# fishaudio/fish-diffusion

Measured on NVIDIA H100. Metric: mel_frames_per_sec_100step_ddpm, higher is better.
Workload: dtype f32 (3x fp16 split-product wgmma, fp32 accumulate)

## Files before the change

### fish_diffusion_b200/csrc/fd_common.cuh

```cuda
#pragma once
#include <cuda_runtime.h>
#include <cuda_fp16.h>
#include <cuda_bf16.h>
#include <stdint.h>

#define FD_F16 0
#define FD_BF16 1
#define FD_SINGLE 0x10

#define FD_MAX_SEG 16

#define FD_EPI_LINEAR 0
#define FD_EPI_GATE 1
#define FD_EPI_RES_SKIP 2
#define FD_EPI_MAG 3
#define FD_EPI_GATE_BWD 4

#define FD_ACT_NONE 0
#define FD_ACT_RELU 1
#define FD_ACT_LRELU 2
#define FD_ACT_GELU 3

struct FdSeg {
  int src;
// ... 123 lines not shown
  const float sg = fd_sigmoid(g), th = fd_tanh(f);
  dg = dz * th * sg * (1.f - sg);
  df = dz * sg * (1.f - th * th);
}

__device__ __forceinline__ void fd_split2(float a, float b, int prec, uint32_t& hi2, uint32_t& lo2) {
  if (prec == FD_F16) {
    asm("cvt.rn.satfinite.f16x2.f32 %0, %1, %2;" : "=r"(hi2) : "f"(b), "f"(a));
    const float2 hf = __half22float2(*reinterpret_cast<const __half2*>(&hi2));
    asm("cvt.rn.satfinite.f16x2.f32 %0, %1, %2;" : "=r"(lo2) : "f"(b - hf.y), "f"(a - hf.x));
  } else {
    asm("cvt.rn.satfinite.bf16x2.f32 %0, %1, %2;" : "=r"(hi2) : "f"(b), "f"(a));
    const float ha = __uint_as_float(hi2 << 16), hb = __uint_as_float(hi2 & 0xffff0000u);
    asm("cvt.rn.satfinite.bf16x2.f32 %0, %1, %2;" : "=r"(lo2) : "f"(b - hb), "f"(a - ha));
  }
}

template <int V>
__device__ __forceinline__ void fd_store_planes(uint16_t* planes, size_t plane_elems, size_t off,
                                                const float (&y)[V], int prec) {
  uint32_t hi[V / 2], lo[V / 2];
#pragma unroll
  for (int i = 0; i < V / 2; ++i) fd_split2(y[2 * i], y[2 * i + 1], prec, hi[i], lo[i]);
  if (V == 4) {
    *reinterpret_cast<uint2*>(planes + off) = make_uint2(hi[0], hi[1]);
    *reinterpret_cast<uint2*>(planes + plane_elems + off) = make_uint2(lo[0], lo[1]);
  } else {
    *reinterpret_cast<uint4*>(planes + off) = make_uint4(hi[0], hi[1], hi[2 % (V / 2)], hi[3 % (V / 2)]);
    *reinterpret_cast<uint4*>(planes + plane_elems + off) = make_uint4(lo[0], lo[1], lo[2 % (V / 2)], lo[3 % (V / 2)]);
  }
}

template <int V>
__device__ __forceinline__ void fd_load_planes(const uint16_t* planes, size_t plane_elems, size_t off,
                                               float (&y)[V], int prec) {
  uint32_t hi[4], lo[4];
  if (V == 4) {
    const uint2 a = *reinterpret_cast<const uint2*>(planes + off);
    const uint2 b = *reinterpret_cast<const uint2*>(planes + plane_elems + off);
    hi[0] = a.x; hi[1] = a.y; lo[0] = b.x; lo[1] = b.y;
  } else {
    const uint4 a = *reinterpret_cast<const uint4*>(planes + off);
    const uint4 b = *reinterpret_cast<const uint4*>(planes + plane_elems + off);
    hi[0] = a.x; hi[1] = a.y; hi[2] = a.z; hi[3] = a.w; lo[0] = b.x; lo[1] = b.y; lo[2] = b.z; lo[3] = b.w;
  }
#pragma unroll
  for (int i = 0; i < V / 2; ++i) fd_combine2(hi[i], lo[i], prec, y[2 * i], y[2 * i + 1]);
}

__device__ __forceinline__ void fd_load_hi8(const uint16_t* planes, size_t off, float (&y)[8], int prec) {
  const uint4 a = *reinterpret_cast<const uint4*>(planes + off);
  const uint32_t w[4] = {a.x, a.y, a.z, a.w};
#pragma unroll
  for (int i = 0; i < 4; ++i) {
    y[2 * i] = fd_h2f((uint16_t)(w[i] & 0xffff), prec);
    y[2 * i + 1] = fd_h2f((uint16_t)(w[i] >> 16), prec);
  }
}

template <int V>
__device__ __forceinline__ void fd_load_f32(const float* p, float (&y)[V]) {
#pragma unroll
  for (int i = 0; i < V; i += 4) {
    float4 q = *reinterpret_cast<const float4*>(p + i);
    y[i] = q.x; y[i + 1] = q.y; y[i + 2] = q.z; y[i + 3] = q.w;
  }
}
template <int V>
__device__ __forceinline__ void fd_store_f32(float* p, const float (&y)[V]) {
#pragma unroll
  for (int i = 0; i < V; i += 4)
    *reinterpret_cast<float4*>(p + i) = make_float4(y[i], y[i + 1], y[i + 2], y[i + 3]);
}

template <typename I>
struct FdRows {
  I item;
  int t0, dt, nrows;
  __device__ __forceinline__ I row(const FdTapGemm& p, int r) const { return item + (I)min(t0 + r * dt, p.T - 1); }
};
// ... 55 lines not shown
    for (int i = 0; i < V; ++i) a[r][i] = (a[r][i] * p.acc_scale + bias[i] + pre[r][i]) * p.post_scale;
  if (p.out_f32 != nullptr && p.out_accum) {
#pragma unroll
    for (int r = 0; r < R; ++r) {
      float v[V];
      fd_load_f32<V>(p.out_f32 + off[r], v);
#pragma unroll
      for (int i = 0; i < V; ++i) a[r][i] += v[i];
    }
  }
  const float slope = p.act == FD_ACT_NONE ? 1.f : p.act == FD_ACT_RELU ? 0.f : p.act_slope;
#pragma unroll
  for (int r = 0; r < R; ++r) {
    if (r >= rw.nrows) break;
    if ((masked >> r) & 1u) {
#pragma unroll
      for (int i = 0; i < V; ++i) a[r][i] = 0.f;
    }
    if (p.out_f32 != nullptr) fd_store_f32<V>(p.out_f32 + off[r], a[r]);
    if (p.out_planes != nullptr) {
      float v[V];
      if (p.act == FD_ACT_GELU) {
#pragma unroll
        for (int i = 0; i < V; ++i) v[i] = fd_gelu(a[r][i] * p.planes_scale);
      } else {
#pragma unroll
        for (int i = 0; i < V; ++i) v[i] = fd_act(a[r][i] * p.planes_scale, slope);
      }
      fd_store_planes<V>(p.out_planes, plane, off[r], v, prec);
    }
  }
}

template <int R, int V, int PREC, typename I>
__device__ __forceinline__ void fd_epi_res_skip(const FdTapGemm& p, const FdRows<I>& rw, int n, bool is_res,
                                                const float (&a)[R][V], const float (&bias)[V]) {
  const int prec = PREC < 0 ? p.prec : PREC;
  const size_t plane = (size_t)p.B * p.T * p.C;
  const I cn = (I)(is_res ? n : n - p.C);
  I off[R];
#pragma unroll
  for (int r = 0; r < R; ++r) off[r] = rw.row(p, r) * (I)p.C + cn;
  if (is_res) {
    if (p.last_layer) return;
    float x[R][V];
#pragma unroll
    for (int r = 0; r < R; ++r) fd_load_planes<V>(p.x_planes, plane, off[r], x[r], prec);
    uint16_t* const xo = p.x_out_planes != nullptr ? p.x_out_planes : p.x_planes;
#pragma unroll
    for (int r = 0; r < R; ++r) {
      if (r >= rw.nrows) break;
#pragma unroll
      for (int i = 0; i < V; ++i) x[r][i] = (x[r][i] + (a[r][i] * p.acc_scale + bias[i])) * 0.70710678118654752440f;
      fd_store_planes<V>(xo, plane, off[r], x[r], prec);
    }
  } else {
    float sk[R][V];
    if (!p.first_layer) {
#pragma unroll
      for (int r = 0; r < R; ++r) fd_load_f32<V>(p.skip_f32 + off[r], sk[r]);
    }
#pragma unroll
    for (int r = 0; r < R; ++r) {
      if (r >= rw.nrows) break;
      float y[V];
#pragma unroll
      for (int i = 0; i < V; ++i) {
        y[i] = a[r][i] * p.acc_scale + bias[i];
        if (!p.first_layer) y[i] += sk[r][i];
      }
      if (p.last_layer) {
#pragma unroll
        for (int i = 0; i < V; ++i) y[i] *= p.skip_scale;
        fd_store_planes<V>(p.skip_planes, plane, off[r], y, prec);
      } else {
        fd_store_f32<V>(p.skip_f32 + off[r], y);
      }
    }
  }
}

template <int V>
__device__ __forceinline__ void fd_epi_gate(const FdTapGemm& p, int t, float (&g)[V], float (&f)[V], float (&z)[V],
                                            const float (&bias)[2][V], const float (&add)[2][V],
                                            const float (&lo)[2][V], const float (&hi)[2][V]) {
#pragma unroll
  for (int i = 0; i < V; ++i) {
    g[i] = g[i] * p.acc_scale + bias[0][i];
    f[i] = f[i] * p.acc_scale + bias[1][i];
  }
  if (p.addend != nullptr) {
#pragma unroll
    for (int i = 0; i < V; ++i) { g[i] += add[0][i]; f[i] += add[1][i]; }
  }
  if (t < p.dil) {
#pragma unroll
    for (int i = 0; i < V; ++i) { g[i] -= lo[0][i]; f[i] -= lo[1][i]; }
  }
  if (t + p.dil >= p.T) {
#pragma unroll
    for (int i = 0; i < V; ++i) { g[i] -= hi[0][i]; f[i] -= hi[1][i]; }
  }
#pragma unroll
  for (int i = 0; i < V; ++i) z[i] = fd_sigmoid(g[i]) * fd_tanh(f[i]);
}

template <int V>
struct FdColSums {
  float all[2][V], lo[2][V], hi[2][V];
};

template <int R, int V, int PREC, typename I>
// ... 120 lines not shown
```

### fish_diffusion_b200/csrc/fd_tapgemm_simt.cu

```cuda
#include "fd_common.cuh"

namespace {

constexpr int BM = 128;
constexpr int BK = 16;
constexpr int APITCH = BM + 4;

template <int RUN, int EPI>
__global__ void __launch_bounds__(256) fd_tapgemm_simt_kernel(const FdTapGemm p) {
  constexpr int BN = 2 * RUN;
  constexpr int TXC = RUN / 4;
  constexpr int TYC = 256 / TXC;
  constexpr int RM = BM / TYC;
  constexpr int BPITCH = BN + 4;

  __shared__ float As[BK][APITCH];
  __shared__ float Bs[BK][BPITCH];

  const int tid = threadIdx.x;
  const int tx = tid % TXC, ty = tid / TXC;
  const int tiles_t = (p.T + BM - 1) / BM;
  const int m_tile = blockIdx.x;
  const int b = m_tile / tiles_t;
  const int t0 = (m_tile % tiles_t) * BM;
  const int j = blockIdx.y;

  int run0, run1;
  if (EPI == FD_EPI_GATE || EPI == FD_EPI_MAG) {
    run0 = fd_gate_col(p, j * RUN);
    run1 = run0 + p.gate_tile / 2;
  } else {
    run0 = j * BN;
    run1 = run0 + RUN;
  }

  float acc[RM][8];
#pragma unroll
  for (int r = 0; r < RM; ++r)
#pragma unroll
    for (int c = 0; c < 8; ++c) acc[r][c] = 0.f;

  const size_t w_plane = (size_t)p.n_total * p.k_total;
  int koff = 0;
  for (int s = 0; s < p.num_seg; ++s) {
    const FdSeg sg = p.seg[s];
    const uint16_t* src = p.src[sg.src];
    const size_t a_plane = (size_t)p.src_ps[sg.src];
    const size_t a_rs = (size_t)p.src_rs[sg.src], a_bs = (size_t)p.src_bs[sg.src];
    for (int k0 = 0; k0 < sg.k_len; k0 += BK) {
      {
        const int row = tid % BM, kh = tid / BM;
        const int t = t0 + row + sg.shift;
        float v[8];
        const int kk = k0 + kh * 8;
        if (t >= 0 && t < p.T && t0 + row < p.T && kk < sg.k_len) {
          const size_t off = (size_t)b * a_bs + (size_t)t * a_rs + sg.c_off + kk;
          if (p.single) fd_load_hi8(src, off, v, p.prec);
          else fd_load_planes<8>(src, a_plane, off, v, p.prec);
        } else {
#pragma unroll
          for (int i = 0; i < 8; ++i) v[i] = 0.f;
        }
#pragma unroll
        for (int i = 0; i < 8; ++i) As[kh * 8 + i][row] = v[i];
      }
// ... 79 lines not shown
          float a[1][4] = {{acc[r][4 * h], acc[r][4 * h + 1], acc[r][4 * h + 2], acc[r][4 * h + 3]}};
          fd_epi_gate_bwd<1, 4, -1>(p, FdRows<size_t>{(size_t)b * p.T, tr + r, 1, 1}, n, a, s);
        }
        fd_gate_bwd_colsums<TXC>(p, s, t0 < p.dil, t0 + BM + p.dil > p.T, tid % 32 < TXC && n < p.n_total, b, n);
      } else {
        if (n >= p.n_total) continue;
#pragma unroll
        for (int r = 0; r < RM; ++r) {
          if (r >= nrows) break;
          float bias[4];
#pragma unroll
          for (int i = 0; i < 4; ++i) bias[i] = p.bias != nullptr ? p.bias[(size_t)b * p.bias_bstride + n + i] : 0.f;
          float a[1][4] = {{acc[r][4 * h], acc[r][4 * h + 1], acc[r][4 * h + 2], acc[r][4 * h + 3]}};
          const FdRows<size_t> row{(size_t)b * p.T, tr + r, 1, 1};
          if constexpr (EPI == FD_EPI_LINEAR) fd_epi_linear<1, 4, -1>(p, row, n, a, bias);
          else fd_epi_res_skip<1, 4, -1>(p, row, n, n < p.C, a, bias);
        }
      }
    }
  }
}

template <int RUN>
int launch_run(const FdTapGemm& p, cudaStream_t stream) {
  const int tiles_t = (p.T + BM - 1) / BM;
  dim3 grid(p.B * tiles_t, 1, 1), block(256);
  if (p.epi == FD_EPI_GATE) {
    grid.y = (p.n_total / 2 + RUN - 1) / RUN;
    fd_tapgemm_simt_kernel<RUN, FD_EPI_GATE><<<grid, block, 0, stream>>>(p);
  } else if (p.epi == FD_EPI_MAG) {
    grid.y = (p.n_total / 2 + RUN - 1) / RUN;
    fd_tapgemm_simt_kernel<RUN, FD_EPI_MAG><<<grid, block, 0, stream>>>(p);
  } else if (p.epi == FD_EPI_RES_SKIP) {
    grid.y = (p.n_total + 2 * RUN - 1) / (2 * RUN);
    fd_tapgemm_simt_kernel<RUN, FD_EPI_RES_SKIP><<<grid, block, 0, stream>>>(p);
  } else if (p.epi == FD_EPI_GATE_BWD) {
    grid.y = (p.n_total + 2 * RUN - 1) / (2 * RUN);
    fd_tapgemm_simt_kernel<RUN, FD_EPI_GATE_BWD><<<grid, block, 0, stream>>>(p);
  } else {
    grid.y = (p.n_total + 2 * RUN - 1) / (2 * RUN);
    fd_tapgemm_simt_kernel<RUN, FD_EPI_LINEAR><<<grid, block, 0, stream>>>(p);
  }
  FD_CHECK_CUDA(cudaGetLastError());
  return 0;
}

constexpr int WG_R = 64, WG_C = 64, WG_T = 16;

__global__ void __launch_bounds__(256) fd_wgrad_simt_kernel(const FdWgradK p, const uint16_t* row0,
                                                            const uint16_t* row1, const uint16_t* col0,
                                                            const uint16_t* col1, int prec, int single) {
  static_assert(WG_R == WG_C, "rows and columns share the staging code");
  __shared__ __align__(16) float Rs[WG_T][WG_R + 4];
  __shared__ __align__(16) float Cs[WG_T][WG_C + 4];
  const int tid = threadIdx.x;
  const int s = blockIdx.z, r0 = blockIdx.y * WG_R, c0 = blockIdx.x * WG_C;

  const bool is_col = tid >= 128;
  const int grp = tid % 8, tl = (tid % 128) / 8;
  const int i = (is_col ? c0 : r0) + grp * 8;
  const uint16_t* src = nullptr;
  int C = 0, ch = 0, shift = 0;
  if (!is_col) {
    for (int g = 0; g < p.num_row_seg; ++g)
      if (i >= p.row_start[g] && i < p.row_start[g] + p.row_width[g]) {
        src = p.row_src[g] == 0 ? row0 : row1;
        C = p.row_C[p.row_src[g]]; ch = p.row_coff[g] + (i - p.row_start[g]);
// ... 94 lines not shown
```

### fish_diffusion_b200/csrc/fd_tapgemm_tc.cu

```cuda
#include <cuda.h>
#include "fd_common.cuh"
#include "fd_host.h"
#include "fd_tc_ptx.cuh"

namespace {

constexpr int BLOCK_M = 128;

template <int BLOCK_N, int BLOCK_K, int EPI, int NPL>
struct Cfg {
  static constexpr bool PP = EPI == FD_EPI_GATE || EPI == FD_EPI_RES_SKIP;
  static constexpr int ROWS = PP ? 64 : BLOCK_M;
  static constexpr int A_BYTES = ROWS * BLOCK_K * 2;
  static constexpr int W_BYTES = BLOCK_N * BLOCK_K * 2;
  static constexpr int GROUP = BLOCK_K >= 64 || PP ? 1 : 64 / BLOCK_K;
  static constexpr int SUB_BYTES = NPL * (A_BYTES + W_BYTES);
  static constexpr int STAGE_BYTES = GROUP * SUB_BYTES;
  static constexpr int TX_BYTES = SUB_BYTES;
  static constexpr int SWIZZLE_BYTES = BLOCK_K * 2;
  static constexpr uint32_t SWIZZLE_MODE = swizzle_mode_for(SWIZZLE_BYTES);
  static constexpr uint32_t SBO = 8 * SWIZZLE_BYTES;
  static constexpr int BIAS_FLOATS = (EPI == FD_EPI_GATE ? 3 : 1) * BLOCK_N;
  static constexpr int BIAS_TOTAL = (PP ? 2 : 1) * BIAS_FLOATS;
  static constexpr int NUM_STAGES = fd_tc_frame_stages(STAGE_BYTES, BIAS_TOTAL);
  static constexpr int SMEM_BYTES = fd_tc_frame_bytes(NUM_STAGES, STAGE_BYTES, BIAS_TOTAL);
  static_assert(NUM_STAGES >= 2, "pipeline needs at least two stages");
  static_assert(SMEM_BYTES <= FD_TC_SMEM_BUDGET, "shared memory");
};

template <int BLOCK_N, int EPI>
__device__ __forceinline__ void stage_bias(const FdTapGemm& p, int b, int n0, float* bias_s, int i0, int step) {
  if (EPI == FD_EPI_GATE) {
    const size_t bo = (size_t)b * p.gbias_bstride + n0;
    for (int i = i0; i < BLOCK_N; i += step) {
      bias_s[i] = p.gbias_full[bo + i];
      bias_s[BLOCK_N + i] = p.gbias_lo[bo + i];
      bias_s[2 * BLOCK_N + i] = p.gbias_hi[bo + i];
    }
  } else {
    for (int i = i0; i < BLOCK_N; i += step)
      bias_s[i] = p.bias ? p.bias[(size_t)b * p.bias_bstride + n0 + i] : 0.f;
  }
}
template <int EPI>
__device__ __forceinline__ long long bias_key(const FdTapGemm& p, int b, int n0) {
  return EPI == FD_EPI_GATE ? (long long)b * p.gbias_bstride + n0 : (long long)b * p.bias_bstride + n0;
}

template <int BLOCK_N, int EPI, int PREC>
__device__ __forceinline__ void tile_epilogue(const FdTapGemm& p, const float* acc, int b, int n_tile, int rw0,
                                              const float* bias_s, uint32_t my_scratch, int lane) {
  const int n0 = n_tile * BLOCK_N;
  if constexpr (EPI == FD_EPI_GATE || EPI == FD_EPI_MAG) {
    constexpr int HALF = BLOCK_N / 2;
    const uint32_t sb = smem_u32(bias_s);
    const int r = lane >> 1, sub = lane & 1;
    const int t = rw0 + r;
    const bool valid = t < p.T;
    const bool e_lo = t < p.dil, e_hi = t + p.dil >= p.T;
    const bool edge_any = __any_sync(0xffffffffu, valid && (e_lo || e_hi));
    const size_t zplane = (size_t)p.B * p.T * p.C, zrow = ((size_t)b * p.T + t) * p.C + (size_t)n_tile * HALF;
    const size_t yplane = (size_t)p.B * p.T * p.n_total, yrow = ((size_t)b * p.T + t) * p.n_total;
#pragma unroll
    for (int c = 0; c < HALF; c += 16) {
      frag_to_scratch<16>(my_scratch, acc, c, 0, lane);
      frag_to_scratch<16>(my_scratch, acc, HALF + c, 16, lane);
      __syncwarp();
      float g[8], f[8];
      {
        const float4 g0 = scratch_ld4(my_scratch, r, 2 * sub), g1 = scratch_ld4(my_scratch, r, 2 * sub + 1);
        const float4 f0 = scratch_ld4(my_scratch, r, 4 + 2 * sub), f1 = scratch_ld4(my_scratch, r, 5 + 2 * sub);
        g[0] = g0.x; g[1] = g0.y; g[2] = g0.z; g[3] = g0.w; g[4] = g1.x; g[5] = g1.y; g[6] = g1.z; g[7] = g1.w;
        f[0] = f0.x; f[1] = f0.y; f[2] = f0.z; f[3] = f0.w; f[4] = f1.x; f[5] = f1.y; f[6] = f1.z; f[7] = f1.w;
      }
      __syncwarp();
      const int cc = c + 8 * sub;
      if (valid) {
        if (EPI == FD_EPI_MAG) {
          fd_epi_mag<8, PREC>(p, b, t, n_tile * HALF + cc, g, f);
        } else {
          float add[2][8], bias[2][8], lo[2][8], hi[2][8], z[8];
          if (p.addend != nullptr) {
#pragma unroll
            for (int h = 0; h < 2; ++h) ldcs_f32(p.addend + yrow + n0 + h * HALF + cc, add[h]);
          }
#pragma unroll
          for (int h = 0; h < 2; ++h) lds_f32(sb + 4u * (h * HALF + cc), bias[h]);
          if (edge_any) {
#pragma unroll
            for (int h = 0; h < 2; ++h)
              if (e_lo) lds_f32(sb + 4u * (BLOCK_N + h * HALF + cc), lo[h]);
#pragma unroll
            for (int h = 0; h < 2; ++h)
              if (e_hi) lds_f32(sb + 4u * (2 * BLOCK_N + h * HALF + cc), hi[h]);
          }
          fd_epi_gate<8>(p, t, g, f, z, bias, add, lo, hi);
          if (p.y_planes != nullptr) {
            const int ng = p.gate_tile == BLOCK_N ? n0 + cc : fd_gate_col(p, n_tile * HALF + cc);
            fd_store_planes<8>(p.y_planes, yplane, yrow + ng, g, PREC);
            fd_store_planes<8>(p.y_planes, yplane, yrow + ng + p.gate_tile / 2, f, PREC);
          }
          fd_store_planes<8>(p.out_planes, zplane, zrow + cc, z, PREC);
        }
      }
    }
  } else if constexpr (BLOCK_N >= 64) {
    const uint32_t bias_addr = smem_u32(bias_s);
    const int j4 = (lane & 7) * 4, rsub = lane >> 3;
    const int rbase = rw0 + rsub;
    const FdRows<uint32_t> rows{(uint32_t)b * (uint32_t)p.T, rbase, 4,
                                rbase < p.T ? min(4, (p.T - rbase + 3) / 4) : 0};
#pragma unroll
    for (int c = 0; c < BLOCK_N; c += 32) {
      const int col = c + j4;
      const int n = n0 + col;
      frag_to_scratch<32>(my_scratch, acc, c, 0, lane);
      __syncwarp();
      float a[4][4];
#pragma unroll
      for (int r = 0; r < 4; ++r) {
        const float4 x = scratch_ld4(my_scratch, 4 * r + rsub, lane & 7);
        a[r][0] = x.x; a[r][1] = x.y; a[r][2] = x.z; a[r][3] = x.w;
      }
      __syncwarp();
      if constexpr (EPI == FD_EPI_GATE_BWD) {
        FdColSums<4> s{};
        fd_epi_gate_bwd<4, 4, PREC>(p, rows, n, a, s);
        fd_gate_bwd_colsums<8>(p, s, rw0 < p.dil, rw0 + 16 + p.dil > p.T, rsub == 0, b, n);
      } else {
        float bias[4];
        lds_f32(bias_addr + 4u * col, bias);
        if constexpr (EPI == FD_EPI_RES_SKIP) fd_epi_res_skip<4, 4, PREC>(p, rows, n, n0 < p.C, a, bias);
        else fd_epi_linear<4, 4, PREC>(p, rows, n, a, bias);
      }
    }
  } else {
    static_assert(EPI == FD_EPI_LINEAR, "narrow tiles: LINEAR only");
    constexpr int PER = BLOCK_N / 2;
    frag_to_scratch<BLOCK_N>(my_scratch, acc, 0, 0, lane);
    __syncwarp();
    const int r = lane >> 1, sub = lane & 1;
    float v[PER];
#pragma unroll
    for (int q4 = 0; q4 < PER / 4; ++q4) {
      const float4 x = scratch_ld4(my_scratch, r, sub * (PER / 4) + q4);
      v[4 * q4] = x.x; v[4 * q4 + 1] = x.y; v[4 * q4 + 2] = x.z; v[4 * q4 + 3] = x.w;
    }
    __syncwarp();
    const int t = rw0 + r;
    const FdRows<uint32_t> row{(uint32_t)b * (uint32_t)p.T, t, 1, t < p.T ? 1 : 0};
#pragma unroll
    for (int h = 0; h < PER / 8; ++h) {
      const int cc = sub * PER + h * 8;
      float a[1][8], bias[8];
#pragma unroll
      for (int i = 0; i < 8; ++i) a[0][i] = v[h * 8 + i];
      lds_f32(smem_u32(bias_s) + 4u * cc, bias);
      fd_epi_linear<1, 8, PREC>(p, row, n0 + cc, a, bias);
    }
  }
}

template <int BLOCK_N, int BLOCK_K, int EPI, int PREC, int NPL>
__global__ void __launch_bounds__(FD_TC_THREADS, 1)
fd_tapgemm_tc_kernel(const __grid_constant__ CUtensorMap tm_src0, const __grid_constant__ CUtensorMap tm_src1,
                     const __grid_constant__ CUtensorMap tm_w, const FdTapGemm p) {
// ... 48 lines not shown

  consumer_regs();
  const int wg = warp / 4;
  const int wq = warp % 4;
  const uint32_t my_scratch = smem_u32(f.scratch) + warp * FD_TC_SCRATCH_WARP_BYTES;
  float* bias_s = f.bias;
  float acc[BLOCK_N / 2];
  long long staged_key = -1;
  for (int tile = blockIdx.x; tile < num_tiles; tile += gridDim.x) {
    const int m_tile = tile / num_n_tiles;
    const int n_tile = (tile % num_n_tiles + m_tile) % num_n_tiles;
    const int b = m_tile / tiles_t, t0 = (m_tile % tiles_t) * BLOCK_M;
    const int n0 = n_tile * BLOCK_N;

    if (EPI == FD_EPI_LINEAR && bias_key<EPI>(p, b, n0) != staged_key) {
      staged_key = bias_key<EPI>(p, b, n0);
      named_bar_sync<1, FD_TC_CONSUMER_THREADS>();
      stage_bias<BLOCK_N, EPI>(p, b, n0, bias_s, threadIdx.x, FD_TC_CONSUMER_THREADS);
      named_bar_sync<1, FD_TC_CONSUMER_THREADS>();
    }

    ring_mainloop(acc, ring, total_k_blocks, C::GROUP, lane, [&](int stage, int nb) {
      for (int g = 0; g < nb; ++g) {
        const uint32_t st = smem_u32(f.ring + stage * C::STAGE_BYTES + g * C::SUB_BYTES);
        const uint32_t wg_a = wg * 64 * C::SWIZZLE_BYTES;
        const uint64_t a_hi = make_smem_desc(st + wg_a, 16, C::SBO, C::SWIZZLE_MODE);
        const uint64_t a_lo = make_smem_desc(st + C::A_BYTES + wg_a, 16, C::SBO, C::SWIZZLE_MODE);
        const uint64_t w_hi = make_smem_desc(st + NPL * C::A_BYTES, 16, C::SBO, C::SWIZZLE_MODE);
        const uint64_t w_lo = make_smem_desc(st + NPL * C::A_BYTES + C::W_BYTES, 16, C::SBO, C::SWIZZLE_MODE);
        split_mma<MMA, NPL, BLOCK_K / 16, 32>(acc, a_hi, a_lo, w_hi, w_lo);
      }
    });

    tile_epilogue<BLOCK_N, EPI, PREC>(p, acc, b, n_tile, t0 + wg * 64 + wq * 16, bias_s, my_scratch, lane);
  }
}

template <int BLOCK_N, int BLOCK_K, int EPI, int PREC, int NPL>
__global__ void __launch_bounds__(FD_TC_THREADS, 1)
fd_tapgemm_pp_kernel(const __grid_constant__ CUtensorMap tm_src0, const __grid_constant__ CUtensorMap tm_src1,
                     const __grid_constant__ CUtensorMap tm_w, const FdTapGemm p) {
  using C = Cfg<BLOCK_N, BLOCK_K, EPI, NPL>;
  static_assert(C::PP && C::GROUP == 1, "ping-pong schedule: GATE / RES_SKIP, one k-block per stage");
  using MMA = Wgmma<BLOCK_N, PREC>;
  extern __shared__ uint8_t smem_raw[];
  const TcFrame f = tc_frame(smem_raw, C::NUM_STAGES, C::STAGE_BYTES, C::BIAS_TOTAL);

  const int warp = threadIdx.x / 32;
  const int lane = threadIdx.x % 32;
  const int rank = (int)cluster_ctarank();
  const int pair = blockIdx.x / 2, num_pairs = gridDim.x / 2;

  const int tiles_t = (p.T + 63) / 64;
  const int num_m_tiles = p.B * tiles_t;
  const int num_n_tiles = p.n_total / BLOCK_N;
  const int num_units = (num_m_tiles + 1) / 2 * num_n_tiles;
  int total_k_blocks = 0;
  for (int sI = 0; sI < p.num_seg; ++sI) total_k_blocks += p.seg[sI].k_len / BLOCK_K;

  tc_prologue<true>(f, C::NUM_STAGES, 2 * 4, &tm_src0, &tm_src1, &tm_w);

  if (warp >= FD_TC_PRODUCER_WARP) {
    producer_regs();
    if (warp == FD_TC_PRODUCER_WARP && lane == 0) {
      Ring ring{f.full, f.empty, C::NUM_STAGES};
      for (int u = pair; u < num_units; u += num_pairs) {
        const int m_pair = u / num_n_tiles;
        const int n_tile = (u % num_n_tiles + m_pair) % num_n_tiles;
        const int m_tile = min(2 * m_pair + rank, num_m_tiles - 1);
        const int b = m_tile / tiles_t, t0 = (m_tile % tiles_t) * 64;
        const int n0 = n_tile * BLOCK_N;
        SegCursor sc;
#pragma unroll 1
        for (int kb = 0; kb < total_k_blocks; ++kb) {
          ring.wait_empty();
          uint8_t* st = f.ring + ring.stage * C::STAGE_BYTES;
          mbar_expect_tx(ring.full_bar(), C::TX_BYTES);
          const FdSeg sg = p.seg[sc.s];
          tma_load_4d(st, sg.src == 0 ? &tm_src0 : &tm_src1, ring.full_bar(), sg.c_off + sc.k0, t0 + sg.shift, b, 0);
          tma_load_3d_multicast(st + NPL * C::A_BYTES + rank * (NPL * C::W_BYTES / 2), &tm_w, ring.full_bar(),
                                sc.koff + sc.k0 + p.w_kshift, n0 + (NPL == 1 ? rank * (BLOCK_N / 2) : 0),
                                NPL == 2 ? rank : 0, 0x3);
          sc.next(BLOCK_K, sg.k_len);
          ring.next();
        }
      }
    }
  } else {
    consumer_regs();
    const int wg = warp / 4;
    const int wq = warp % 4;
    const uint32_t my_scratch = smem_u32(f.scratch) + warp * FD_TC_SCRATCH_WARP_BYTES;
    float* my_bias = f.bias + wg * C::BIAS_FLOATS;
    float acc[BLOCK_N / 2];
    PingPong turn(f.full, f.empty, C::NUM_STAGES, total_k_blocks, wg);
    long long staged_key = -1;
    for (int u = pair + wg * num_pairs; u < num_units; u += 2 * num_pairs) {
      const int m_pair = u / num_n_tiles;
      const int n_tile = (u % num_n_tiles + m_pair) % num_n_tiles;
      const int m_tile = 2 * m_pair + rank;
      const bool valid = m_tile < num_m_tiles;
      const int b = m_tile / tiles_t, t0 = (m_tile % tiles_t) * 64;
      const int n0 = n_tile * BLOCK_N;

      if (valid && bias_key<EPI>(p, b, n0) != staged_key) {
        staged_key = bias_key<EPI>(p, b, n0);
        wg == 0 ? named_bar_sync<3, 128>() : named_bar_sync<4, 128>();
        stage_bias<BLOCK_N, EPI>(p, b, n0, my_bias, threadIdx.x % 128, 128);
        wg == 0 ? named_bar_sync<3, 128>() : named_bar_sync<4, 128>();
      }

      turn.mainloop(acc, u == pair, u + num_pairs < num_units, lane, [&](int stage) {
        const uint32_t st = smem_u32(f.ring + stage * C::STAGE_BYTES);
        const uint64_t a_hi = make_smem_desc(st, 16, C::SBO, C::SWIZZLE_MODE);
        const uint64_t a_lo = make_smem_desc(st + C::A_BYTES, 16, C::SBO, C::SWIZZLE_MODE);
        const uint64_t w_hi = make_smem_desc(st + NPL * C::A_BYTES, 16, C::SBO, C::SWIZZLE_MODE);
        const uint64_t w_lo = make_smem_desc(st + NPL * C::A_BYTES + C::W_BYTES, 16, C::SBO, C::SWIZZLE_MODE);
        split_mma<MMA, NPL, BLOCK_K / 16, 32>(acc, a_hi, a_lo, w_hi, w_lo);
      });

      if (valid) tile_epilogue<BLOCK_N, EPI, PREC>(p, acc, b, n_tile, t0 + wq * 16, my_bias, my_scratch, lane);
    }
  }
  __syncwarp();
  cluster_sync();
}

template <int BLOCK_T>
struct GateTCfg {
  static constexpr int BLOCK_K = 32;
  static constexpr int ROW_BYTES = BLOCK_K * 2;
  static constexpr int ACT_ROWS = BLOCK_T + 16;
  static constexpr int MAX_DIL = (ACT_ROWS - BLOCK_T) / 2;
  static constexpr int ACT_PLANE = ACT_ROWS * ROW_BYTES;
  static constexpr int W_PLANE = 64 * ROW_BYTES;
  static constexpr int W_OFF = 2 * ACT_PLANE;
  static constexpr int STAGE_BYTES = W_OFF + 3 * 2 * W_PLANE;
  static constexpr uint32_t SWIZZLE_MODE = swizzle_mode_for(ROW_BYTES);
  static constexpr uint32_t SBO = 8 * ROW_BYTES;
  static constexpr int NUM_STAGES = fd_tc_frame_stages(STAGE_BYTES, 0);
  static constexpr int SMEM_BYTES = fd_tc_frame_bytes(NUM_STAGES, STAGE_BYTES, 0);
  static_assert(ACT_ROWS <= 256, "one TMA box per plane");
  static_assert(ACT_PLANE % 512 == 0 && STAGE_BYTES % 1024 == 0, "planes start on 64 B swizzle atoms");
  static_assert(NUM_STAGES >= 3, "ring depth");
  static_assert(SMEM_BYTES <= FD_TC_SMEM_BUDGET, "shared memory");
};

template <int BLOCK_T, int PREC>
__device__ __forceinline__ void gate_t_epilogue(const FdTapGemm& p, const float* acc, int b, int t0, int ch,
                                                uint32_t my_scratch, int lane) {
  const int half = p.gate_tile / 2;
  const int e = lane >> 2, q4 = lane & 3;
  const int n_g = fd_gate_col(p, ch) + e, n_f = n_g + half;
  const size_t bo = (size_t)b * p.gbias_bstride;
// ... 153 lines not shown

template <int BLOCK_T, int PREC>
int launch_gate_t(const FdTapGemm& p, cudaStream_t stream) {
  using C = GateTCfg<BLOCK_T>;
  CUtensorMap tmx, tmw;
  int rc = planes_map(&tmx, p.src[0], p.src_C[0], p.T, p.B, p.src_rs[0], p.src_bs[0], p.src_ps[0], C::BLOCK_K,
                      BLOCK_T + 2 * p.dil, 1, "gate_t x");
  if (rc) return rc;
  const int half = p.gate_tile / 2;
  const cuuint64_t K = (cuuint64_t)p.k_total;
  const cuuint64_t dims[5] = {K, 8, 2, (cuuint64_t)p.n_total / 8, 2};
  const cuuint64_t strides[4] = {K * 2, (cuuint64_t)half * K * 2, 8 * K * 2, (cuuint64_t)p.n_total * K * 2};
  const cuuint32_t box[5] = {(cuuint32_t)C::BLOCK_K, 8, 2, 4, 2};
  rc = encode_tiled(&tmw, p.w, 5, dims, strides, box, "gate_t w");
  if (rc) return rc;
  const int units = p.B * ((p.T + BLOCK_T - 1) / BLOCK_T) * (p.n_total / 128);
  return fd_tc_launch<fd_gate_t_kernel<BLOCK_T, PREC>>(C::SMEM_BYTES, 2 * units, stream, false, 2, tmx, tmw, p);
}

template <int BLOCK_N, int BLOCK_K, int EPI, int PREC, int NPL>
int launch_inst(const FdTapGemm& p, cudaStream_t stream) {
  using C = Cfg<BLOCK_N, BLOCK_K, EPI, NPL>;
  CUtensorMap tm0, tm1, tmw;
  int rc = planes_map(&tm0, p.src[0], p.src_C[0], p.T, p.B, p.src_rs[0], p.src_bs[0], p.src_ps[0], BLOCK_K, C::ROWS,
                      NPL, "tapgemm src0");
  if (rc) return rc;
  if (p.src[1] != nullptr) {
    rc = planes_map(&tm1, p.src[1], p.src_C[1], p.T, p.B, p.src_rs[1], p.src_bs[1], p.src_ps[1], BLOCK_K, C::ROWS, NPL,
                    "tapgemm src1");
    if (rc) return rc;
  } else {
    tm1 = tm0;
  }
  const int m_tiles = p.B * ((p.T + C::ROWS - 1) / C::ROWS), n_tiles = p.n_total / BLOCK_N;
  if constexpr (C::PP) {
    rc = weights_map(&tmw, p.w, p.n_total, p.k_total, BLOCK_K, NPL == 2 ? BLOCK_N : BLOCK_N / 2, 1, "tapgemm w");
    if (rc) return rc;
    return fd_tc_launch<fd_tapgemm_pp_kernel<BLOCK_N, BLOCK_K, EPI, PREC, NPL>>(
        C::SMEM_BYTES, 2 * ((m_tiles + 1) / 2 * n_tiles), stream, false, 2, tm0, tm1, tmw, p);
  } else {
    rc = weights_map(&tmw, p.w, p.n_total, p.k_total, BLOCK_K, BLOCK_N, NPL, "tapgemm w");
    if (rc) return rc;
    return fd_tc_launch<fd_tapgemm_tc_kernel<BLOCK_N, BLOCK_K, EPI, PREC, NPL>>(C::SMEM_BYTES, m_tiles * n_tiles,
                                                                              stream, false, 1, tm0, tm1, tmw, p);
  }
}

template <int BLOCK_N, int BLOCK_K, int EPI>
int launch_cfg(const FdTapGemm& p, cudaStream_t stream) {
  if (p.single) {
    return p.prec == FD_F16 ? launch_inst<BLOCK_N, BLOCK_K, EPI, FD_F16, 1>(p, stream)
                            : launch_inst<BLOCK_N, BLOCK_K, EPI, FD_BF16, 1>(p, stream);
  }
  return p.prec == FD_F16 ? launch_inst<BLOCK_N, BLOCK_K, EPI, FD_F16, 2>(p, stream)
                          : launch_inst<BLOCK_N, BLOCK_K, EPI, FD_BF16, 2>(p, stream);
}

template <int BLOCK_N, int BLOCK_K>
int launch_epi(const FdTapGemm& p, cudaStream_t stream) {
  if (p.epi == FD_EPI_GATE) return launch_cfg<BLOCK_N, BLOCK_K, FD_EPI_GATE>(p, stream);
  if (p.epi == FD_EPI_MAG) return launch_cfg<BLOCK_N, BLOCK_K, FD_EPI_MAG>(p, stream);
  if (p.epi == FD_EPI_RES_SKIP) return launch_cfg<BLOCK_N, BLOCK_K, FD_EPI_RES_SKIP>(p, stream);
  if (p.epi == FD_EPI_GATE_BWD) return launch_cfg<BLOCK_N, BLOCK_K, FD_EPI_GATE_BWD>(p, stream);
  return launch_cfg<BLOCK_N, BLOCK_K, FD_EPI_LINEAR>(p, stream);
}

void pick_cfg(const FdTapGemm& p, int* bn, int* bk) {
  *bn = 0; *bk = 0;
  bool all64 = true, all32 = true, all16 = true;
  for (int s = 0; s < p.num_seg; ++s) {
    if (p.seg[s].c_off % 16 != 0) return;
    all64 &= p.seg[s].k_len % 64 == 0;
    all32 &= p.seg[s].k_len % 32 == 0;
    all16 &= p.seg[s].k_len % 16 == 0;
  }
  const int k = all64 ? 64 : all32 ? 32 : all16 ? 16 : 0;
  if (k == 0) return;
  const int npl = p.single ? 1 : 2;
  auto wavenet_bk = [&](int n) {
    return fd_tc_frame_stages(npl * (64 + n) * 64 * 2, 2 * (p.epi == FD_EPI_GATE ? 3 : 1) * n) < 3 ? 32 : 64;
  };
  if (p.epi == FD_EPI_GATE || p.epi == FD_EPI_MAG) {
    const int n = p.gate_tile;
    if ((n != 256 && n != 128) || p.n_total % n != 0 || k != 64) return;
    *bn = n; *bk = p.epi == FD_EPI_GATE ? wavenet_bk(n) : 64;
    return;
  }
  int n = 256;
  while (n >= 16 && (p.n_total % n != 0 || (p.epi == FD_EPI_RES_SKIP && p.C % n != 0))) n >>= 1;
  if (n < 16) return;
  if (k == 64) {
    if (n < 64) return;
    *bn = n; *bk = p.epi == FD_EPI_RES_SKIP ? wavenet_bk(n) : 64;
  } else if (k == 32) {
    if (p.epi != FD_EPI_LINEAR || n < 32) return;
    *bn = n > 64 ? 64 : n; *bk = 32;
  } else {
    if (p.epi != FD_EPI_LINEAR) return;
    *bn = n > 32 ? 32 : n; *bk = 16;
  }
}

}

int fd_tapgemm_tc_supported(const FdTapGemm& p) {
  int bn, bk;
  pick_cfg(p, &bn, &bk);
  if (bn == 0) return 0;
  for (int s = 0; s < 2; ++s)
    if (p.src[s] != nullptr && (p.src_rs[s] % 8 != 0 || p.src_bs[s] % 8 != 0 || p.src_ps[s] % 8 != 0)) return 0;
  if (p.k_total % 8 != 0) return 0;
  return 1;
}

int fd_tapgemm_tc_launch(const FdTapGemm& p, cudaStream_t stream) {
  int bn, bk;
  pick_cfg(p, &bn, &bk);
  const long long width = p.epi == FD_EPI_GATE_BWD ? 2ll * p.n_total : p.n_total;
  FD_REQUIRE((long long)p.B * p.T * width < (1ll << 32),
             "tapgemm(tc): B*T*%lld = %lld exceeds the 32-bit element offsets of the epilogue", width,
             (long long)p.B * p.T * width);
// ... 32 lines not shown
```

Before: 22760.

## Prefetch res/skip epilogue inputs before MMA and skip dead residual tiles on last layer

```diff
diff --git a/fish_diffusion_b200/csrc/fd_common.cuh b/fish_diffusion_b200/csrc/fd_common.cuh
--- a/fish_diffusion_b200/csrc/fd_common.cuh
+++ b/fish_diffusion_b200/csrc/fd_common.cuh
@@ -179,20 +179,31 @@
 }
 
 template <int V>
-__device__ __forceinline__ void fd_load_planes(const uint16_t* planes, size_t plane_elems, size_t off,
-                                               float (&y)[V], int prec) {
-  uint32_t hi[4], lo[4];
-  if (V == 4) {
+__device__ __forceinline__ void fd_load_plane_words(const uint16_t* planes, size_t plane_elems, size_t off,
+                                                    uint32_t (&w)[V]) {
+  static_assert(V == 4 || V == 8, "4 or 8 channels");
+  if constexpr (V == 4) {
     const uint2 a = *reinterpret_cast<const uint2*>(planes + off);
     const uint2 b = *reinterpret_cast<const uint2*>(planes + plane_elems + off);
-    hi[0] = a.x; hi[1] = a.y; lo[0] = b.x; lo[1] = b.y;
+    w[0] = a.x; w[1] = a.y; w[2] = b.x; w[3] = b.y;
   } else {
     const uint4 a = *reinterpret_cast<const uint4*>(planes + off);
     const uint4 b = *reinterpret_cast<const uint4*>(planes + plane_elems + off);
-    hi[0] = a.x; hi[1] = a.y; hi[2] = a.z; hi[3] = a.w; lo[0] = b.x; lo[1] = b.y; lo[2] = b.z; lo[3] = b.w;
-  }
-#pragma unroll
-  for (int i = 0; i < V / 2; ++i) fd_combine2(hi[i], lo[i], prec, y[2 * i], y[2 * i + 1]);
+    w[0] = a.x; w[1] = a.y; w[2] = a.z; w[3] = a.w; w[4] = b.x; w[5] = b.y; w[6] = b.z; w[7] = b.w;
+  }
+}
+template <int V>
+__device__ __forceinline__ void fd_combine_words(const uint32_t (&w)[V], int prec, float (&y)[V]) {
+#pragma unroll
+  for (int i = 0; i < V / 2; ++i) fd_combine2(w[i], w[V / 2 + i], prec, y[2 * i], y[2 * i + 1]);
+}
+
+template <int V>
+__device__ __forceinline__ void fd_load_planes(const uint16_t* planes, size_t plane_elems, size_t off,
+                                               float (&y)[V], int prec) {
+  uint32_t w[V];
+  fd_load_plane_words<V>(planes, plane_elems, off, w);
+  fd_combine_words<V>(w, prec, y);
 }
 
 __device__ __forceinline__ void fd_load_hi8(const uint16_t* planes, size_t off, float (&y)[8], int prec) {
@@ -314,52 +325,73 @@
   }
 }
 
+__host__ __device__ inline int fd_res_skip_first_col(const FdTapGemm& p) { return p.last_layer ? p.C : 0; }
+
+template <int R, int V, typename I>
+__device__ __forceinline__ void fd_res_skip_load(const FdTapGemm& p, const FdRows<I>& rw, int n, bool is_res,
+                                                 uint32_t (&in)[R][V]) {
+  const size_t plane = (size_t)p.B * p.T * p.C;
+  const I cn = (I)(is_res ? n : n - p.C);
+  if (is_res) {
+#pragma unroll
+    for (int r = 0; r < R; ++r) fd_load_plane_words<V>(p.x_planes, plane, rw.row(p, r) * (I)p.C + cn, in[r]);
+  } else if (!p.first_layer) {
+#pragma unroll
+    for (int r = 0; r < R; ++r) {
+      float sk[V];
+      fd_load_f32<V>(p.skip_f32 + rw.row(p, r) * (I)p.C + cn, sk);
+#pragma unroll
+      for (int i = 0; i < V; ++i) in[r][i] = __float_as_uint(sk[i]);
+    }
+  }
+}
+
+template <int R, int V, int PREC, typename I>
+__device__ __forceinline__ void fd_res_skip_store(const FdTapGemm& p, const FdRows<I>& rw, int n, bool is_res,
+                                                  const uint32_t (&in)[R][V], const float (&a)[R][V],
+                                                  const float (&bias)[V]) {
+  const int prec = PREC < 0 ? p.prec : PREC;
+  const size_t plane = (size_t)p.B * p.T * p.C;
+  const I cn = (I)(is_res ? n : n - p.C);
+  if (is_res) {
+    uint16_t* const xo = p.x_out_planes != nullptr ? p.x_out_planes : p.x_planes;
+#pragma unroll
+    for (int r = 0; r < R; ++r) {
+      if (r >= rw.nrows) break;
+      float x[V];
+      fd_combine_words<V>(in[r], prec, x);
+#pragma unroll
+      for (int i = 0; i < V; ++i) x[i] = (x[i] + (a[r][i] * p.acc_scale + bias[i])) * 0.70710678118654752440f;
+      fd_store_planes<V>(xo, plane, rw.row(p, r) * (I)p.C + cn, x, prec);
+    }
+  } else {
+#pragma unroll
+    for (int r = 0; r < R; ++r) {
+      if (r >= rw.nrows) break;
+      const I off = rw.row(p, r) * (I)p.C + cn;
+      float y[V];
+#pragma unroll
+      for (int i = 0; i < V; ++i) {
+        y[i] = a[r][i] * p.acc_scale + bias[i];
+        if (!p.first_layer) y[i] += __uint_as_float(in[r][i]);
+      }
+      if (p.last_layer) {
+#pragma unroll
+        for (int i = 0; i < V; ++i) y[i] *= p.skip_scale;
+        fd_store_planes<V>(p.skip_planes, plane, off, y, prec);
+      } else {
+        fd_store_f32<V>(p.skip_f32 + off, y);
+      }
+    }
+  }
+}
+
 template <int R, int V, int PREC, typename I>
 __device__ __forceinline__ void fd_epi_res_skip(const FdTapGemm& p, const FdRows<I>& rw, int n, bool is_res,
                                                 const float (&a)[R][V], const float (&bias)[V]) {
-  const int prec = PREC < 0 ? p.prec : PREC;
-  const size_t plane = (size_t)p.B * p.T * p.C;
-  const I cn = (I)(is_res ? n : n - p.C);
-  I off[R];
-#pragma unroll
-  for (int r = 0; r < R; ++r) off[r] = rw.row(p, r) * (I)p.C + cn;
-  if (is_res) {
-    if (p.last_layer) return;
-    float x[R][V];
-#pragma unroll
-    for (int r = 0; r < R; ++r) fd_load_planes<V>(p.x_planes, plane, off[r], x[r], prec);
-    uint16_t* const xo = p.x_out_planes != nullptr ? p.x_out_planes : p.x_planes;
-#pragma unroll
-    for (int r = 0; r < R; ++r) {
-      if (r >= rw.nrows) break;
-#pragma unroll
-      for (int i = 0; i < V; ++i) x[r][i] = (x[r][i] + (a[r][i] * p.acc_scale + bias[i])) * 0.70710678118654752440f;
-      fd_store_planes<V>(xo, plane, off[r], x[r], prec);
-    }
-  } else {
-    float sk[R][V];
-    if (!p.first_layer) {
-#pragma unroll
-      for (int r = 0; r < R; ++r) fd_load_f32<V>(p.skip_f32 + off[r], sk[r]);
-    }
-#pragma unroll
-    for (int r = 0; r < R; ++r) {
-      if (r >= rw.nrows) break;
-      float y[V];
-#pragma unroll
-      for (int i = 0; i < V; ++i) {
-        y[i] = a[r][i] * p.acc_scale + bias[i];
-        if (!p.first_layer) y[i] += sk[r][i];
-      }
-      if (p.last_layer) {
-#pragma unroll
-        for (int i = 0; i < V; ++i) y[i] *= p.skip_scale;
-        fd_store_planes<V>(p.skip_planes, plane, off[r], y, prec);
-      } else {
-        fd_store_f32<V>(p.skip_f32 + off[r], y);
-      }
-    }
-  }
+  uint32_t in[R][V];
+  fd_res_skip_load<R, V>(p, rw, n, is_res, in);
+  fd_res_skip_store<R, V, PREC>(p, rw, n, is_res, in, a, bias);
 }
 
 template <int V>
diff --git a/fish_diffusion_b200/csrc/fd_tapgemm_simt.cu b/fish_diffusion_b200/csrc/fd_tapgemm_simt.cu
--- a/fish_diffusion_b200/csrc/fd_tapgemm_simt.cu
+++ b/fish_diffusion_b200/csrc/fd_tapgemm_simt.cu
@@ -30,7 +30,7 @@
     run0 = fd_gate_col(p, j * RUN);
     run1 = run0 + p.gate_tile / 2;
   } else {
-    run0 = j * BN;
+    run0 = (EPI == FD_EPI_RES_SKIP ? fd_res_skip_first_col(p) : 0) + j * BN;
     run1 = run0 + RUN;
   }
 
@@ -176,7 +176,7 @@
     grid.y = (p.n_total / 2 + RUN - 1) / RUN;
     fd_tapgemm_simt_kernel<RUN, FD_EPI_MAG><<<grid, block, 0, stream>>>(p);
   } else if (p.epi == FD_EPI_RES_SKIP) {
-    grid.y = (p.n_total + 2 * RUN - 1) / (2 * RUN);
+    grid.y = (p.n_total - fd_res_skip_first_col(p) + 2 * RUN - 1) / (2 * RUN);
     fd_tapgemm_simt_kernel<RUN, FD_EPI_RES_SKIP><<<grid, block, 0, stream>>>(p);
   } else if (p.epi == FD_EPI_GATE_BWD) {
     grid.y = (p.n_total + 2 * RUN - 1) / (2 * RUN);
diff --git a/fish_diffusion_b200/csrc/fd_tapgemm_tc.cu b/fish_diffusion_b200/csrc/fd_tapgemm_tc.cu
--- a/fish_diffusion_b200/csrc/fd_tapgemm_tc.cu
+++ b/fish_diffusion_b200/csrc/fd_tapgemm_tc.cu
@@ -47,9 +47,22 @@
   return EPI == FD_EPI_GATE ? (long long)b * p.gbias_bstride + n0 : (long long)b * p.bias_bstride + n0;
 }
 
-template <int BLOCK_N, int EPI, int PREC>
+__device__ __forceinline__ FdRows<uint32_t> coalesced_rows(const FdTapGemm& p, int b, int rw0, int lane) {
+  const int rbase = rw0 + (lane >> 3);
+  return {(uint32_t)b * (uint32_t)p.T, rbase, 4, rbase < p.T ? min(4, (p.T - rbase + 3) / 4) : 0};
+}
+__device__ __forceinline__ int coalesced_col(int c, int lane) { return c + (lane & 7) * 4; }
+
+template <int BLOCK_N>
+constexpr int RS_AHEAD = BLOCK_N == 256 ? 3 : BLOCK_N / 32;
+__device__ __forceinline__ void res_skip_chunk_load(const FdTapGemm& p, const FdRows<uint32_t>& rows, int n0, int chunk,
+                                                    int lane, uint32_t (&in)[4][4]) {
+  fd_res_skip_load<4, 4>(p, rows, n0 + coalesced_col(32 * chunk, lane), n0 < p.C, in);
+}
+
+template <int BLOCK_N, int EPI, int PREC, class In>
 __device__ __forceinline__ void tile_epilogue(const FdTapGemm& p, const float* acc, int b, int n_tile, int rw0,
-                                              const float* bias_s, uint32_t my_scratch, int lane) {
+                                              const float* bias_s, uint32_t my_scratch, int lane, In&& in) {
   const int n0 = n_tile * BLOCK_N;
   if constexpr (EPI == FD_EPI_GATE || EPI == FD_EPI_MAG) {
     constexpr int HALF = BLOCK_N / 2;
@@ -106,13 +119,11 @@
     }
   } else if constexpr (BLOCK_N >= 64) {
     const uint32_t bias_addr = smem_u32(bias_s);
-    const int j4 = (lane & 7) * 4, rsub = lane >> 3;
-    const int rbase = rw0 + rsub;
-    const FdRows<uint32_t> rows{(uint32_t)b * (uint32_t)p.T, rbase, 4,
-                                rbase < p.T ? min(4, (p.T - rbase + 3) / 4) : 0};
+    const int rsub = lane >> 3;
+    const FdRows<uint32_t> rows = coalesced_rows(p, b, rw0, lane);
 #pragma unroll
     for (int c = 0; c < BLOCK_N; c += 32) {
-      const int col = c + j4;
+      const int col = coalesced_col(c, lane);
       const int n = n0 + col;
       frag_to_scratch<32>(my_scratch, acc, c, 0, lane);
       __syncwarp();
@@ -130,8 +141,14 @@
       } else {
         float bias[4];
         lds_f32(bias_addr + 4u * col, bias);
-        if constexpr (EPI == FD_EPI_RES_SKIP) fd_epi_res_skip<4, 4, PREC>(p, rows, n, n0 < p.C, a, bias);
-        else fd_epi_linear<4, 4, PREC>(p, rows, n, a, bias);
+        if constexpr (EPI == FD_EPI_RES_SKIP) {
+          constexpr int AHEAD = RS_AHEAD<BLOCK_N>;
+          const int ci = c / 32;
+          fd_res_skip_store<4, 4, PREC>(p, rows, n, n0 < p.C, in[ci % AHEAD], a, bias);
+          if (ci + AHEAD < BLOCK_N / 32) res_skip_chunk_load(p, rows, n0, ci + AHEAD, lane, in[ci % AHEAD]);
+        } else {
+          fd_epi_linear<4, 4, PREC>(p, rows, n, a, bias);
+        }
       }
     }
   } else {
@@ -246,7 +263,7 @@
       }
     });
 
-    tile_epilogue<BLOCK_N, EPI, PREC>(p, acc, b, n_tile, t0 + wg * 64 + wq * 16, bias_s, my_scratch, lane);
+    tile_epilogue<BLOCK_N, EPI, PREC>(p, acc, b, n_tile, t0 + wg * 64 + wq * 16, bias_s, my_scratch, lane, 0);
   }
 }
 
@@ -267,7 +284,8 @@
 
   const int tiles_t = (p.T + 63) / 64;
   const int num_m_tiles = p.B * tiles_t;
-  const int num_n_tiles = p.n_total / BLOCK_N;
+  const int n_first = EPI == FD_EPI_RES_SKIP ? fd_res_skip_first_col(p) / BLOCK_N : 0;
+  const int num_n_tiles = p.n_total / BLOCK_N - n_first;
   const int num_units = (num_m_tiles + 1) / 2 * num_n_tiles;
   int total_k_blocks = 0;
   for (int sI = 0; sI < p.num_seg; ++sI) total_k_blocks += p.seg[sI].k_len / BLOCK_K;
@@ -280,7 +298,7 @@
       Ring ring{f.full, f.empty, C::NUM_STAGES};
       for (int u = pair; u < num_units; u += num_pairs) {
         const int m_pair = u / num_n_tiles;
-        const int n_tile = (u % num_n_tiles + m_pair) % num_n_tiles;
+        const int n_tile = n_first + (u % num_n_tiles + m_pair) % num_n_tiles;
         const int m_tile = min(2 * m_pair + rank, num_m_tiles - 1);
         const int b = m_tile / tiles_t, t0 = (m_tile % tiles_t) * 64;
         const int n0 = n_tile * BLOCK_N;
@@ -309,13 +327,21 @@
     float acc[BLOCK_N / 2];
     PingPong turn(f.full, f.empty, C::NUM_STAGES, total_k_blocks, wg);
     long long staged_key = -1;
+    uint32_t in[EPI == FD_EPI_RES_SKIP ? RS_AHEAD<BLOCK_N> : 1][4][4];
     for (int u = pair + wg * num_pairs; u < num_units; u += 2 * num_pairs) {
       const int m_pair = u / num_n_tiles;
-      const int n_tile = (u % num_n_tiles + m_pair) % num_n_tiles;
+      const int n_tile = n_first + (u % num_n_tiles + m_pair) % num_n_tiles;
       const int m_tile = 2 * m_pair + rank;
       const bool valid = m_tile < num_m_tiles;
       const int b = m_tile / tiles_t, t0 = (m_tile % tiles_t) * 64;
       const int n0 = n_tile * BLOCK_N;
+      if constexpr (EPI == FD_EPI_RES_SKIP) {
+        if (valid) {
+          const FdRows<uint32_t> rows = coalesced_rows(p, b, t0 + wq * 16, lane);
+#pragma unroll
+          for (int c = 0; c < RS_AHEAD<BLOCK_N>; ++c) res_skip_chunk_load(p, rows, n0, c, lane, in[c]);
+        }
+      }
 
       if (valid && bias_key<EPI>(p, b, n0) != staged_key) {
         staged_key = bias_key<EPI>(p, b, n0);
@@ -333,7 +359,7 @@
         split_mma<MMA, NPL, BLOCK_K / 16, 32>(acc, a_hi, a_lo, w_hi, w_lo);
       });
 
-      if (valid) tile_epilogue<BLOCK_N, EPI, PREC>(p, acc, b, n_tile, t0 + wq * 16, my_bias, my_scratch, lane);
+      if (valid) tile_epilogue<BLOCK_N, EPI, PREC>(p, acc, b, n_tile, t0 + wq * 16, my_bias, my_scratch, lane, in);
     }
   }
   __syncwarp();
@@ -553,7 +579,8 @@
   } else {
     tm1 = tm0;
   }
-  const int m_tiles = p.B * ((p.T + C::ROWS - 1) / C::ROWS), n_tiles = p.n_total / BLOCK_N;
+  const int m_tiles = p.B * ((p.T + C::ROWS - 1) / C::ROWS);
+  const int n_tiles = (p.n_total - (EPI == FD_EPI_RES_SKIP ? fd_res_skip_first_col(p) : 0)) / BLOCK_N;
   if constexpr (C::PP) {
     rc = weights_map(&tmw, p.w, p.n_total, p.k_total, BLOCK_K, NPL == 2 ? BLOCK_N : BLOCK_N / 2, 1, "tapgemm w");
     if (rc) return rc;
@@ -581,7 +608,10 @@
 int launch_epi(const FdTapGemm& p, cudaStream_t stream) {
   if (p.epi == FD_EPI_GATE) return launch_cfg<BLOCK_N, BLOCK_K, FD_EPI_GATE>(p, stream);
   if (p.epi == FD_EPI_MAG) return launch_cfg<BLOCK_N, BLOCK_K, FD_EPI_MAG>(p, stream);
-  if (p.epi == FD_EPI_RES_SKIP) return launch_cfg<BLOCK_N, BLOCK_K, FD_EPI_RES_SKIP>(p, stream);
+  if (p.epi == FD_EPI_RES_SKIP) {
+    if constexpr (BLOCK_N <= 128) return launch_cfg<BLOCK_N, BLOCK_K, FD_EPI_RES_SKIP>(p, stream);
+    FD_REQUIRE(false, "tapgemm(tc): no %d x %d RES_SKIP instantiation", BLOCK_N, BLOCK_K);
+  }
   if (p.epi == FD_EPI_GATE_BWD) return launch_cfg<BLOCK_N, BLOCK_K, FD_EPI_GATE_BWD>(p, stream);
   return launch_cfg<BLOCK_N, BLOCK_K, FD_EPI_LINEAR>(p, stream);
 }
@@ -607,7 +637,7 @@
     *bn = n; *bk = p.epi == FD_EPI_GATE ? wavenet_bk(n) : 64;
     return;
   }
-  int n = 256;
+  int n = p.epi == FD_EPI_RES_SKIP && p.single ? 128 : 256;
   while (n >= 16 && (p.n_total % n != 0 || (p.epi == FD_EPI_RES_SKIP && p.C % n != 0))) n >>= 1;
   if (n < 16) return;
   if (k == 64) {
```

Result: faster. 23080, median of 6 (+1.4%).
